# ut-vision/Rot-MVGaze

Measured on AMD Instinct MI355X. Metric: multi-view samples/sec (fwd+bwd), BxVx3x224x224, higher is better.
Workload: dtype f32; 1 GPU; C3: ResNet-50, V=4, B=128 per GPU, 3x224x224, fwd+loss+bwd; backbone=ResNet-50, views=4, batch_per_gpu=128, global_batch=128, image=3x224x224, parallelism=dp1, weights=random init, seed 0 (kaiming-normal convs, default Linear), rccl_ranks=1, step_launch=eager: every kernel queued from Python

## Files before the change

include/rotmvgaze.h:

```cpp
#ifndef ROTMVGAZE_H
#define ROTMVGAZE_H

#include <stddef.h>
#include <stdint.h>

#ifdef __cplusplus
extern "C" {
#endif

#define MVG_ABI_VERSION 13

int mvg_abi_version(void);
const char *mvg_last_error(void);
int mvg_device_cus(void);
int mvg_set_scratch(void *ptr, size_t bytes, void *stream);
size_t mvg_scratch_bytes(void);
void *mvg_stream_create_low_priority(void);
int mvg_set_reserved_cus(int n);

enum {
  MVG_K_CONV_FPROP = 0, MVG_K_CONV_DGRAD = 1, MVG_K_CONV_WGRAD = 2, MVG_K_WGRAD_REDUCE = 3,
  MVG_K_BN_FINALIZE = 4, MVG_K_BN_APPLY = 5, MVG_K_BN_BWD_REDUCE = 6, MVG_K_BN_BWD_APPLY = 7,
  MVG_K_POOL = 8, MVG_K_LAYOUT = 9, MVG_K_LINEAR_FPROP = 10, MVG_K_LINEAR_DGRAD = 11,
  MVG_K_LINEAR_WGRAD = 12, MVG_K_ROTCAT = 13, MVG_K_COLSUM = 14, MVG_K_LOSS = 15,
// ... 310 lines not shown
                            float *dz_out, float *mx, const float *gamma, float *dy_sinv, void *stream);
int mvg_bn_bwd_apply_split(const float *g, const float *y, const float *mean, const float *invstd, const float *gamma,
                           const float *s1, const float *s2, const float *relu_scale, const float *relu_shift,
                           int groups, int64_t rows_per_group, int c, void *dy_sp, const float *mx, float *dy_sinv,
                           int dy_sinv_ready, void *stream);
int mvg_bn_relu_maxpool_fwd_split(const float *y, const float *scale, const float *shift, void *pooled_sp,
                                  uint8_t *argmax, int groups, int n_per_group, int h, int w, int c, int ho, int wo,
                                  void *stream);
int mvg_avgpool_fwd_split(const void *x_sp, float *y, int n, int hw, int c, void *stream);
int mvg_act_scales(const void *items_dev, int n, float *slots, int n_slots, void *stream);
int mvg_bn_apply_split_scaled(const float *y, const float *scale, const float *shift, const void *residual, int residual_sp,
                              const float *res_scale, const float *res_shift, const float *res_sinv, int relu, void *out_sp,
                              const float *out_sinv, uint8_t *relu_bits, int groups, int64_t rows_per_group, int c,
                              void *stream);
int mvg_bn_relu_maxpool_fwd_split_scaled(const float *y, const float *scale, const float *shift, void *pooled_sp,
                                         const float *pooled_sinv, uint8_t *argmax, int groups, int n_per_group, int h, int w,
                                         int c, int ho, int wo, void *stream);
int mvg_avgpool_fwd_split_scaled(const void *x_sp, const float *x_sinv, float *y, int n, int hw, int c, void *stream);
int mvg_conv_dgrad_bn_partials_split(const mvg_conv_desc *d);
int mvg_conv_dgrad_split_bnreduce(const mvg_conv_desc *d, const void *dy_sp, const float *dy_sinv, const void *w_crsk_sp,
                                  const float *w_sinv, float *dx, const float *addend, const float *bn_y, const uint8_t *bn_bits,
                                  const float *bn_mean, const float *bn_invstd, const float *relu_scale, const float *relu_shift,
                                  float *partials, float *s1, float *s2, float *dgamma, float *dbeta, int accumulate,
                                  float *mx, const float *bn_gamma, float *dx_dy_sinv, void *stream);
int mvg_conv_dgrad_split_bnapply_bnreduce(const mvg_conv_desc *d, void *dy_sp, const float *dy_sinv, const float *dz, const float *y,
                                          const float *mean, const float *invstd, const float *gamma, const float *un_s1,
                                          const float *un_s2, int64_t rows_per_group, const void *w_crsk_sp, const float *w_sinv,
                                          float *dx, const float *addend, const float *bn_y, const uint8_t *bn_bits,
                                          const float *bn_mean, const float *bn_invstd, const float *relu_scale,
                                          const float *relu_shift, float *partials, float *s1, float *s2, float *dgamma, float *dbeta,
                                          int accumulate, float *mx, const float *bn_gamma, float *dx_dy_sinv, void *stream);
int mvg_conv_fprop_split_stages(const mvg_conv_desc *d);
int mvg_conv_dgrad_split_stages(const mvg_conv_desc *d, int fused_reduce);
int mvg_conv_fprop_split_bnapply(const mvg_conv_desc *d, void *out_sp, const float *out_sinv, const float *bn_y, const float *scale,
                                 const float *shift, const void *residual, int residual_sp, const float *res_scale,
                                 const float *res_shift, const float *res_sinv, uint8_t *relu_bits, const void *w_sp,
                                 const float *w_sinv, float *y, float *stats, void *stream);
int mvg_stem_rowwindow_split(const float *x_nhwc4, void *xw_sp, int64_t images, int h, int w, void *stream);
int mvg_stem_rowwindow_split_nchw(const float *x_nchw, void *xw_sp, int64_t images, int h, int w, void *stream);
int mvg_stem_fprop_split(const mvg_conv_desc *d, const void *xw_sp, const void *w_sp, const float *w_sinv, float *y, float *stats,
                         void *stream);
int mvg_stem_wgrad_splits_split(const mvg_conv_desc *d);
int mvg_stem_wgrad_split(const mvg_conv_desc *d, const void *xw_sp, const void *dy_sp, const float *dy_sinv, float *dw_rw,
                         float *workspace, int splits, int accumulate, void *stream);
int mvg_bn_relu_maxpool_bwd_reduce_split(const float *g_pooled, const uint8_t *argmax, const float *y, const float *mean,
                                         const float *invstd, const float *scale, const float *shift, int groups,
                                         int n_per_group, int h, int w, int c, int ho, int wo, float *s1, float *s2,
                                         float *dgamma, float *dbeta, int accumulate, float *workspace, float *mx, const float *gamma,
                                         float *dy_sinv, void *stream);
int mvg_bn_relu_maxpool_bwd_apply_split(const float *g_pooled, const uint8_t *argmax, const float *y, const float *mean,
                                        const float *invstd, const float *gamma, const float *scale, const float *shift,
                                        const float *s1, const float *s2, int groups, int n_per_group, int h, int w, int c,
                                        int ho, int wo, void *dy_sp, const float *mx, float *dy_sinv, int dy_sinv_ready, void *stream);
int mvg_conv_wgrad_splits_split(const mvg_conv_desc *d);
int mvg_conv_wgrad_split_tile(const mvg_conv_desc *d, int32_t *bm, int32_t *bn, int32_t *incremental);
int mvg_conv_wgrad_split(const mvg_conv_desc *d, const void *x_sp, const void *dy_sp, const float *dy_sinv, float *dw,
                         float *workspace, int splits, int accumulate, void *stream);
int mvg_conv_wgrad_split_slabs(const mvg_conv_desc *d, const void *x_sp, const void *dy_sp, const float *dy_sinv, float *workspace,
                               int splits, void *stream);
int mvg_conv_wgrad_split_xs(const mvg_conv_desc *d, const void *x_sp, const float *x_sinv, const void *dy_sp, const float *dy_sinv,
                            float *dw, float *workspace, int splits, int accumulate, void *stream);
int mvg_conv_wgrad_split_slabs_xs(const mvg_conv_desc *d, const void *x_sp, const float *x_sinv, const void *dy_sp,
                                  const float *dy_sinv, float *workspace, int splits, void *stream);
int mvg_wgrad_reduce_batch(const float *const *host_slabs, float *const *host_dw, const int64_t *host_n, const int32_t *host_splits,
                           const int32_t *host_accumulate, int n, void *stream);

// ... 53 lines not shown
```

rot-mvgaze_amd/_lib.py:

```python
from __future__ import annotations

import ctypes as C
import os

_HERE = os.path.dirname(os.path.abspath(__file__))
LIB_PATH = os.path.join(_HERE, "csrc", "librotmvgaze_hip.so")

K_FAMILIES = 18
ABI_VERSION = 13
SESSION_FP32, SESSION_BF16 = 0, 1


class ConvDesc(C.Structure):
    _fields_ = [(n, C.c_int32) for n in
                ("groups", "n", "h", "w", "cin", "cout", "r", "s", "stride", "pad", "ho", "wo")]

    @classmethod
    def make(cls, groups, n, h, w, cin, cout, k, stride, pad):
        ho = (h + 2 * pad - k) // stride + 1
        wo = (w + 2 * pad - k) // stride + 1
        return cls(groups, n, h, w, cin, cout, k, k, stride, pad, ho, wo)

    @classmethod
    def linear(cls, rows, fin, fout):
# ... 71 lines not shown
    "mvg_bn_apply": (_I, [_P, _P, _P, _P, _P, _P, _I, _P, _I, _I64, _I, _P]),
    "mvg_bn_bwd_reduce": (_I, [_P, _P, _P, _P, _P, _P, _P, _I, _I64, _I, _P, _P, _P, _P, _I, _P, _P, _P]),
    "mvg_split_f32": (_I, [_P, _P, _I64, _F, _P]),
    "mvg_merge_sp": (_I, [_P, _P, _I64, _F, _P]),
    "mvg_split_weights": (_I, [_D, _P, _P, _P, _P, _P, _P]),
    "mvg_weights_prep_batch": (_I, [_P, _I, _I, _I, _P]),
    "mvg_conv_stats_partials_split": (_I, [_D, C.POINTER(C.c_int32)]),
    "mvg_conv_fprop_split": (_I, [_D, _P, _P, _P, _P, _P, _P, _P]),
    "mvg_conv_fprop_split_affine": (_I, [_D, _P, _P, _P, _P, _P, _I, _P, _P, _P, _I, _I, _P]),
    "mvg_conv_dgrad_split": (_I, [_D, _P, _P, _P, _P, _P, _P, _P, _P]),
    "mvg_bn_apply_split": (_I, [_P, _P, _P, _P, _I, _P, _P, _I, _P, _P, _I, _I64, _I, _P]),
    "mvg_bn_bwd_apply_split": (_I, [_P, _P, _P, _P, _P, _P, _P, _P, _P, _I, _I64, _I, _P, _P, _P, _I, _P]),
    "mvg_bn_bwd_reduce_split": (_I, [_P, _P, _P, _P, _P, _P, _P, _I, _I64, _I, _P, _P, _P, _P, _I, _P, _P, _P, _P, _P, _P]),
    "mvg_bn_relu_maxpool_fwd_split": (_I, [_P, _P, _P, _P, _P, _I, _I, _I, _I, _I, _I, _I, _P]),
    "mvg_avgpool_fwd_split": (_I, [_P, _P, _I, _I, _I, _P]),
    "mvg_act_scales": (_I, [_P, _I, _P, _I, _P]),
    "mvg_bn_apply_split_scaled": (_I, [_P, _P, _P, _P, _I, _P, _P, _P, _I, _P, _P, _P, _I, _I64, _I, _P]),
    "mvg_bn_relu_maxpool_fwd_split_scaled": (_I, [_P, _P, _P, _P, _P, _P, _I, _I, _I, _I, _I, _I, _I, _P]),
    "mvg_avgpool_fwd_split_scaled": (_I, [_P, _P, _P, _I, _I, _I, _P]),
    "mvg_conv_wgrad_split_xs": (_I, [_D, _P, _P, _P, _P, _P, _P, _I, _I, _P]),
    "mvg_conv_wgrad_split_slabs_xs": (_I, [_D, _P, _P, _P, _P, _P, _I, _P]),
    "mvg_stem_rowwindow_split": (_I, [_P, _P, _I64, _I, _I, _P]),
    "mvg_stem_rowwindow_split_nchw": (_I, [_P, _P, _I64, _I, _I, _P]),
    "mvg_stem_fprop_split": (_I, [_D, _P, _P, _P, _P, _P, _P]),
    "mvg_stem_wgrad_splits_split": (_I, [_D]),
    "mvg_stem_wgrad_split": (_I, [_D, _P, _P, _P, _P, _P, _I, _I, _P]),
    "mvg_bn_relu_maxpool_bwd_reduce_split": (_I, [_P, _P, _P, _P, _P, _P, _P, _I, _I, _I, _I, _I, _I, _I, _P, _P, _P, _P, _I, _P, _P, _P, _P, _P]),
    "mvg_bn_relu_maxpool_bwd_apply_split": (_I, [_P, _P, _P, _P, _P, _P, _P, _P, _P, _P, _I, _I, _I, _I, _I, _I, _I, _P, _P, _P, _I, _P]),
    "mvg_conv_dgrad_bn_partials_split": (_I, [_D]),
    "mvg_conv_dgrad_split_bnreduce": (_I, [_D, _P, _P, _P, _P, _P, _P, _P, _P, _P, _P, _P, _P, _P, _P, _P, _P, _P, _I, _P, _P, _P, _P]),
    "mvg_conv_dgrad_split_bnapply_bnreduce": (_I, [_D] + [_P] * 9 + [_I64] + [_P] * 15 + [_I, _P, _P, _P, _P]),
    "mvg_conv_fprop_split_stages": (_I, [_D]),
    "mvg_conv_dgrad_split_stages": (_I, [_D, _I]),
    "mvg_conv_fprop_split_bnapply": (_I, [_D] + [_P] * 6 + [_I] + [_P] * 9),
    "mvg_conv_wgrad_splits_split": (_I, [_D]),
    "mvg_conv_wgrad_split_tile": (_I, [_D, C.POINTER(C.c_int32), C.POINTER(C.c_int32), C.POINTER(C.c_int32)]),
    "mvg_conv_wgrad_split": (_I, [_D, _P, _P, _P, _P, _P, _I, _I, _P]),
    "mvg_conv_wgrad_split_slabs": (_I, [_D, _P, _P, _P, _P, _I, _P]),
    "mvg_wgrad_reduce_batch": (_I, [C.POINTER(C.c_void_p), C.POINTER(C.c_void_p), C.POINTER(C.c_int64), C.POINTER(C.c_int32),
                                    C.POINTER(C.c_int32), _I, _P]),
    "mvg_bn_apply_bits": (_I, [_P, _P, _P, _P, _P, _P, _P, _P, _I, _I64, _I, _P]),
    "mvg_bn_bwd_reduce_bits": (_I, [_P, _P, _P, _P, _P, _I, _I64, _I, _P, _P, _P, _P, _I, _P, _P, _P]),
    "mvg_bn_apply_bits_bf16": (_I, [_P, _P, _P, _P, _P, _P, _P, _P, _I, _I64, _I, _P]),
    "mvg_bn_bwd_reduce_bits_bf16": (_I, [_P, _P, _P, _P, _P, _I, _I64, _I, _P, _P, _P, _P, _I, _P, _P, _P]),
    "mvg_bn_bwd_workspace_floats": (C.c_size_t, [_I, _I64, _I]),
    "mvg_bn_bwd_apply": (_I, [_P, _P, _P, _P, _P, _P, _P, _P, _P, _P, _I, _I64, _I, _P, _P, _P]),
    "mvg_maxpool3x3s2_fwd": (_I, [_P, _P, _P, _I, _I, _I, _I, _I, _I, _P]),
    "mvg_maxpool3x3s2_bwd": (_I, [_P, _P, _P, _I, _I, _I, _I, _I, _I, _P]),
    "mvg_bn_relu_maxpool_fwd": (_I, [_P, _P, _P, _P, _P, _I, _I, _I, _I, _I, _I, _I, _P]),
    "mvg_bn_relu_maxpool_bwd_reduce": (_I, [_P, _P, _P, _P, _P, _P, _P, _I, _I, _I, _I, _I, _I, _I, _P, _P, _P, _P, _I, _P,
                                            _P]),
    "mvg_bn_relu_maxpool_bwd_apply": (_I, [_P, _P, _P, _P, _P, _P, _P, _P, _P, _P, _I, _I, _I, _I, _I, _I, _I, _P, _P]),
    "mvg_bn_eval_bwd": (_I, [_P, _P, _P, _P, _P, _P, _P, _P, _P, _F, _I, _I64, _I, _P, _P, _P, _P, _I, _P, _P]),
    "mvg_bn_eval_bwd_workspace_floats": (C.c_size_t, [_I, _I64, _I]),
    "mvg_bn_relu_maxpool_eval_bwd": (_I, [_P, _P, _P, _P, _P, _P, _P, _P, _F, _I, _I, _I, _I, _I, _I, _I, _P, _P, _P, _I, _P,
                                          _P]),
    "mvg_avgpool_fwd": (_I, [_P, _P, _I, _I, _I, _P]),
    "mvg_avgpool_bwd": (_I, [_P, _P, _I, _I, _I, _P]),
    "mvg_nchw_to_nhwc4": (_I, [_P, _P, _I, _I, _I, _I, _P]),
    "mvg_nhwc4_to_nchw": (_I, [_P, _P, _I, _I, _I, _I, _P]),
    "mvg_preprocess_u8hwc": (_I, [_P, _P, _I, _I, _I, _F, _F, _F, _F, _F, _F, _I, _P]),
    "mvg_gaze_lp_loss": (_I, [_P, _P, _I, _I, _P, _P, _P]),
    "mvg_preprocess_u8hwc_resize": (_I, [_P, _P, _I, _I, _I, _I, _I, _F, _F, _F, _F, _F, _F, _I, _P]),
    "mvg_multi_erase_nchw": (_I, [_P, _P, _P, _I, _I, _I, _I, _I, _P]),
    "mvg_augment_u8hwc": (_I, [_P, _P, _P, _P, _P, _P, _P, _I, _I, _I, _I, _F, _F, _F, _F, _F, _F, _I, _P]),
    "mvg_rotation_matrix_2d": (_I, [_P, _P, _I, _I, _P]),
# ... 104 lines not shown
```

rot-mvgaze_amd/csrc/conv_split.hip:

```cpp
#include "bf16_tile.h"
#include "elem.h"

namespace mvg {

typedef _Float16 f16x8 __attribute__((ext_vector_type(8)));

#define SPLIT_ONE(PA, PB, av, bv, acc)                                                                         \
  _Pragma("unroll") for (int i = 0; i < TM; ++i) _Pragma("unroll") for (int j = 0; j < TN; ++j)                \
      acc[i][j] = __builtin_amdgcn_mfma_f32_32x32x16_f16(av[PA][i], bv[PB][j], acc[i][j], 0, 0, 0);
#define SPLIT_PRODUCTS(av, bv, acc) SPLIT_ONE(0, 1, av, bv, acc) SPLIT_ONE(1, 0, av, bv, acc) SPLIT_ONE(0, 0, av, bv, acc)

constexpr int SP_BM = 128, SP_BK = 32;

__global__ __launch_bounds__(256) void split_f32_kernel(const float4 *__restrict__ x, uint4 *__restrict__ out, long long n8, float scale) {
  const long long stride = (long long)gridDim.x * 256;
  for (long long i = (long long)blockIdx.x * 256 + threadIdx.x; i < n8; i += stride) {
    const float4 lo = x[2 * i], hi = x[2 * i + 1];
    const float v[8] = {lo.x * scale, lo.y * scale, lo.z * scale, lo.w * scale, hi.x * scale, hi.y * scale, hi.z * scale, hi.w * scale};
    uint4 q1, q2;
    split2_chunk(v, q1, q2);
    out[2 * i] = q1;
    out[2 * i + 1] = q2;
  }
}
// ... 182 lines not shown
#pragma unroll
        for (int q = 0; q < 2; ++q) {
          const int idx = threadIdx.x + 256 * q, cl = idx >> 3, o8 = idx & 7;
          float v[8];
#pragma unroll
          for (int k = 0; k < 8; ++k) v[k] = tile[o8 * 8 + k][cl];
          *reinterpret_cast<uint4 *>(wt + (long long)(c0 + cl) * cout + o0 + o8 * 8) =
              make_uint4(bf16_pack2(v[0], v[1]), bf16_pack2(v[2], v[3]), bf16_pack2(v[4], v[5]), bf16_pack2(v[6], v[7]));
        }
      }
    }
    return;
  }
  for (long long i = (long long)blockIdx.x * 256 + threadIdx.x; i < total; i += (long long)gridDim.x * 256) {
    const int c = (int)(i % cin_pad);
    const long long t = i / cin_pad;
    const int tap = (int)(t % rs), o = (int)(t / rs);
    const float v = c < cin ? w[((long long)o * rs + tap) * cin + c] : 0.f;
    const __bf16 b = (__bf16)v;
    const unsigned short u = __builtin_bit_cast(unsigned short, b);
    wk[i] = u;
    if (wt) wt[((long long)c * rs + tap) * cout + o] = u;
  }
}

typedef float f32x4 __attribute__((ext_vector_type(4)));

#define SPLIT16_ONE(PA, PB)                                                                       \
  _Pragma("unroll") for (int i = 0; i < TM; ++i) _Pragma("unroll") for (int j = 0; j < TN; ++j)   \
      acc[i][j] = __builtin_amdgcn_mfma_f32_16x16x32_f16(av[PA][i], bv[PB][j], acc[i][j], 0, 0, 0);

__device__ __forceinline__ int sp_row_swz(int R) { return ((R >> 1) & 1) | (((R >> 2) & 1) << 2); }

enum AForm : int { A_DMA = 0, A_DY = 1, A_OUT_SP = 2, A_OUT_AFFINE = 3 };
constexpr int BNA_MAX_C = 512;

__device__ __forceinline__ void unpack8(const float4 (&v)[2], float (&o)[8]) {
  o[0] = v[0].x; o[1] = v[0].y; o[2] = v[0].z; o[3] = v[0].w; o[4] = v[1].x; o[5] = v[1].y; o[6] = v[1].z; o[7] = v[1].w;
}

struct DyFormer {
  static constexpr int TABLES = 5;
  __amdgpu_buffer_rsrc_t rs_dz, rs_y;
  float inv_rows, dsc;
  float4 dzv[2][2], yv[2][2];
  float mu[8], is[8], ga[8], sa[8], sb[8];
  static __device__ __forceinline__ void stage(float *t, const IgemmParams &p, int g, int C, int tid) {
    for (int i = tid; i < C; i += 256) {
      const long long gc = (long long)g * C + i;
      t[i] = p.bna_mean[gc];
      t[C + i] = p.bna_invstd[gc];
      t[2 * C + i] = p.bna_gamma[i];
      t[3 * C + i] = p.bna_s1[gc];
      t[4 * C + i] = p.bna_s2[gc];
    }
  }
  __device__ __forceinline__ DyFormer(const IgemmParams &p, long long grow0, long long rows_per_group, int C)
      : rs_dz(make_rsrc(p.bna_dz + grow0 * C, 4ll * rows_per_group * C)), rs_y(make_rsrc(p.bna_y + grow0 * C, 4ll * rows_per_group * C)),
        inv_rows(p.bna_inv_rows), dsc(1.f / *p.a_sinv) {}
  __device__ __forceinline__ void load(int i, unsigned off) {
    dzv[i][0] = buf_ld16(rs_dz, off);
    dzv[i][1] = buf_ld16(rs_dz, off + 16u);
    yv[i][0] = buf_ld16(rs_y, off);
    yv[i][1] = buf_ld16(rs_y, off + 16u);
  }
  __device__ __forceinline__ void consts(const float *kc, int C) {
    ld8(kc, mu);
// ... 264 lines not shown
static int validate_split(const mvg_conv_desc *d) {
  if (validate(d)) return 2;
  MVG_REQUIRE(d->cin % 32 == 0 && d->cout % 32 == 0, "split conv: cin and cout must be multiples of 32 (got %d, %d)", d->cin,
              d->cout);
  MVG_REQUIRE(d->r * d->s <= 32, "split conv: at most 32 filter taps");
  return 0;
}

static int split_tile_rows(int ncols, int taps, long long rows) { return (ncols < 128 && taps > 1 && rows >= 65536) ? 256 : SP_BM; }

struct SplitPlan { int bm, bn, kt_max; long long tiles; bool pipelined; };
static int split_conv_stages(const SplitPlan &pl) { return (pl.pipelined && pl.bn == 128 && pl.bm == SP_BM) ? 2 : 1; }
static SplitPlan split_plan(int ncols, int taps, long long rows, int groups, bool lin, IgemmClass *cls, int ncls) {
  SplitPlan pl;
  pl.bm = lin ? SP_BM : split_tile_rows(ncols, taps, rows);
  pl.bn = ncols >= 128 ? 128 : 64;
  if (lin && pl.bn == 128 && ncls == 1) {
    const long long t128 = (long long)groups * ceil_div(cls[0].rows_per_group, pl.bm) * ceil_div(ncols, 128);
    if (2 * t128 <= compute_cus()) pl.bn = 64;
  }
  pl.tiles = 0, pl.kt_max = 0;
  for (int i = 0; i < ncls; ++i) {
    IgemmClass &c = cls[i];
    c.mtiles_per_group = ceil_div(c.rows_per_group, pl.bm);
    c.KT = ceil_div(c.ktotal, SP_BK);
    c.tile0 = (int)pl.tiles;
    pl.tiles += (long long)groups * c.mtiles_per_group * ceil_div(ncols, pl.bn);
    pl.kt_max = c.KT > pl.kt_max ? c.KT : pl.kt_max;
  }
  pl.pipelined = pl.tiles <= 2LL * compute_cus() || (pl.tiles <= 4LL * compute_cus() && pl.kt_max >= 48);
  return pl;
}

template <bool DGRAD>
static int launch_igemm_split(IgemmParams &p, hipStream_t st, bool lin, int taps, long long rows, AForm af = A_DMA, bool ranged = false) {
  const SplitPlan pl = split_plan(p.ncols, taps, rows, p.groups, lin, p.cls, p.ncls);
  const int bm = pl.bm, bn = pl.bn;
  const bool pipelined = pl.pipelined;
  p.ntiles = ceil_div(p.ncols, bn);
  p.splits = 1;
  p.sk_tiles = 0;
  p.bn_parts = 0;
  for (int i = 0; i < p.ncls; ++i) {
    IgemmClass &c = p.cls[i];
    c.korder = c.ntaps > 1 ? 1 : 0;
    c.per_div = make_fastdiv((unsigned)(c.ntaps > 0 ? c.ntaps : 1));
    c.unit0 = 0;
    c.part0 = p.bn_parts;
    p.bn_parts += c.mtiles_per_group;
    MVG_REQUIRE((c.ntaps >= 1 || (DGRAD && p.bn_part)) && c.ntaps <= 32 && c.ktotal % SP_BK == 0, "split conv: class shape not covered");
  }
  MVG_REQUIRE(pl.tiles < (1LL << 31), "split conv: grid too large");
  if (pl.tiles <= 0) return 0;
  p.nt_out = (!lin && !(DGRAD && p.cls_step == 2)) ? 1 : 0;
  dim3 grid((unsigned)pl.tiles), block(256);
  if (af != A_DMA) {
    MVG_REQUIRE(!lin && bm == SP_BM && p.ntiles == 1 && p.ncls == 1 && DGRAD == (af == A_DY), "split conv: the operand-forming loaders take one column tile");
    if constexpr (DGRAD) {
      if (bn == 128) hipLaunchKernelGGL((igemm_split16_kernel<128, true, false, 2, 1, A_DY>), grid, block, 0, st, p);
      else hipLaunchKernelGGL((igemm_split16_kernel<64, true, false, 2, 1, A_DY>), grid, block, 0, st, p);
      return check_launch("conv_dgrad_split_bnapply");
    } else {
      if (bn == 128 && af == A_OUT_AFFINE) hipLaunchKernelGGL((igemm_split16_kernel<128, false, false, 2, 1, A_OUT_AFFINE>), grid, block, 0, st, p);
      else if (bn == 128) hipLaunchKernelGGL((igemm_split16_kernel<128, false, false, 2, 1, A_OUT_SP>), grid, block, 0, st, p);
      else if (af == A_OUT_AFFINE) hipLaunchKernelGGL((igemm_split16_kernel<64, false, false, 2, 1, A_OUT_AFFINE>), grid, block, 0, st, p);
      else hipLaunchKernelGGL((igemm_split16_kernel<64, false, false, 2, 1, A_OUT_SP>), grid, block, 0, st, p);
      return check_launch("conv_fprop_split_bnapply");
    }
  }
  if (ranged) {
    MVG_REQUIRE(!DGRAD && !lin && p.out_sp && p.out_absmax, "split conv: the range record goes with a forward that stores sp");
    if constexpr (!DGRAD) {
      if (bm == 256) hipLaunchKernelGGL((igemm_split16_ranged_kernel<64, 4>), grid, block, 0, st, p);
      else if (split_conv_stages(pl) == 2) hipLaunchKernelGGL((igemm_split16_ranged_kernel<128, 2, 2>), grid, block, 0, st, p);
      else if (bn == 128) hipLaunchKernelGGL((igemm_split16_ranged_kernel<128>), grid, block, 0, st, p);
      else hipLaunchKernelGGL((igemm_split16_ranged_kernel<64>), grid, block, 0, st, p);
    }
    return check_launch("conv_fprop_split_ranged");
  }
  if (lin) {
    if (bn == 128 && pipelined) hipLaunchKernelGGL((igemm_split16_kernel<128, DGRAD, true, 2, 2>), grid, block, 0, st, p);
    else if (bn == 128) hipLaunchKernelGGL((igemm_split16_kernel<128, DGRAD, true>), grid, block, 0, st, p);
    else if (pipelined) hipLaunchKernelGGL((igemm_split16_kernel<64, DGRAD, true, 2, 2>), grid, block, 0, st, p);
    else hipLaunchKernelGGL((igemm_split16_kernel<64, DGRAD, true>), grid, block, 0, st, p);
  } else if (bm == 256) hipLaunchKernelGGL((igemm_split16_kernel<64, DGRAD, false, 4>), grid, block, 0, st, p);
  else if (split_conv_stages(pl) == 2) hipLaunchKernelGGL((igemm_split16_kernel<128, DGRAD, false, 2, 2>), grid, block, 0, st, p);
  else if (bn == 128) hipLaunchKernelGGL((igemm_split16_kernel<128, DGRAD>), grid, block, 0, st, p);
  else hipLaunchKernelGGL((igemm_split16_kernel<64, DGRAD>), grid, block, 0, st, p);
  return check_launch(DGRAD ? "conv_dgrad_split" : "conv_fprop_split");
}

}

using namespace mvg;

extern "C" {

int mvg_split_f32(const float *x, void *out_sp, int64_t n, float scale, void *stream) {
  MVG_REQUIRE(x && out_sp && n >= 0 && n % 8 == 0, "split_f32: null argument or n %% 8 != 0");
  MVG_REQUIRE(scale > 0.f, "split_f32: scale must be positive (a power of two keeps the round trip exact)");
  if (n == 0) return 0;
  hipStream_t st = (hipStream_t)stream;
  ProfScope ps(MVG_K_LAYOUT, st, 0.0, (4.0 + SP_BYTES) * (double)n);
  long long blocks = (n / 8 + 255) / 256;
  if (blocks > 8192) blocks = 8192;
  hipLaunchKernelGGL(split_f32_kernel, dim3((unsigned)blocks), dim3(256), 0, st, (const float4 *)x, (uint4 *)out_sp, (long long)(n / 8), scale);
  return check_launch("split_f32");
}

int mvg_split_f32_ranged(const float *x, void *out_sp, int64_t n, float scale, uint32_t *range_word, void *stream) {
  MVG_REQUIRE(x && out_sp && range_word && n >= 0 && n % 8 == 0, "split_f32_ranged: null argument or n %% 8 != 0");
  MVG_REQUIRE(scale > 0.f, "split_f32_ranged: scale must be positive (a power of two keeps the round trip exact)");
  if (n == 0) return 0;
  hipStream_t st = (hipStream_t)stream;
  ProfScope ps(MVG_K_LAYOUT, st, 0.0, (4.0 + SP_BYTES) * (double)n);
  long long blocks = (n / 8 + 255) / 256;
  if (blocks > 8192) blocks = 8192;
  hipLaunchKernelGGL(split_f32_ranged_kernel, dim3((unsigned)blocks), dim3(256), 0, st, (const float4 *)x, (uint4 *)out_sp, (long long)(n / 8), scale,
// ... 211 lines not shown
    p.bna_invstd = bna->invstd;
    p.bna_gamma = bna->gamma;
    p.bna_s1 = bna->s1;
    p.bna_s2 = bna->s2;
    p.bna_inv_rows = 1.0f / (float)bna->rows_per_group;
  }
  if (dgrad_geometry(p, d, SP_BYTES, SP_BYTES, "split conv")) return 2;
  MVG_REQUIRE((long long)d->n * d->h * d->w * d->cin < (1ll << 31), "split conv: a group of dx exceeds 2^31 elements");
  const double flops = 2.0 * d->groups * (double)d->n * d->ho * d->wo * d->cout * d->r * d->s * d->cin;
  const double bytes = (double)SP_BYTES * (d->groups * (double)d->n * d->ho * d->wo * d->cout + (double)d->cout * d->r * d->s * d->cin) +
                       (bnf ? 8.25 : 4.0) * d->groups * (double)d->n * d->h * d->w * d->cin +
                       (bna ? 8.0 : 0.0) * d->groups * (double)d->n * d->ho * d->wo * d->cout;
  const bool lin = d->r == 1 && d->s == 1 && d->h == 1 && d->w == 1;
  ProfScope ps(lin ? MVG_K_LINEAR_DGRAD : MVG_K_CONV_DGRAD, (hipStream_t)stream, flops, bytes);
  if (int e = dgrad_classes(p, d, bnf != nullptr, 4, dx, addend, (hipStream_t)stream)) return e;
  if (p.ncls == 0) return 0;
  return launch_igemm_split<true>(p, (hipStream_t)stream, lin_kernel, d->r * d->s, (long long)d->n * d->h * d->w, bna ? A_DY : A_DMA);
}

int mvg_conv_dgrad_split(const mvg_conv_desc *d, const void *dy_sp, const float *dy_sinv, const void *w_crsk_sp, const float *w_sinv,
                         float *dx, const float *addend, const void *relu_mask_sp, void *stream) {
  MVG_REQUIRE(!relu_mask_sp || d->stride == 1, "dgrad_split: the sp ReLU mask is for stride-1 launches (Linear layers)");
  return dgrad_split_impl(d, dy_sp, dy_sinv, w_crsk_sp, w_sinv, dx, addend, stream, nullptr, relu_mask_sp);
}

int mvg_conv_dgrad_split_stages(const mvg_conv_desc *d, int fused_reduce) {
  if (validate_split(d)) return -1;
  IgemmParams p;
  memset(&p, 0, sizeof(p));
  if (dgrad_geometry(p, d, SP_BYTES, SP_BYTES, "split conv")) return -1;
  DgradDropped dropped;
  dgrad_plan_classes(p, d, fused_reduce != 0, dropped);
  return split_conv_stages(split_plan(p.ncols, d->r * d->s, (long long)d->n * d->h * d->w, p.groups, false, p.cls, p.ncls));
}

int mvg_conv_dgrad_bn_partials_split(const mvg_conv_desc *d) {
  if (validate_split(d)) return -1;
  return dgrad_bn_partials(d, split_tile_rows(d->cin, d->r * d->s, (long long)d->n * d->h * d->w));
}

static int dgrad_split_bnreduce_impl(const char *who, const mvg_conv_desc *d, const void *dy_sp, const float *dy_sinv, const void *w_crsk_sp,
                                     const float *w_sinv, float *dx, const float *addend, const float *bn_y, const uint8_t *bn_bits,
                                     const float *bn_mean, const float *bn_invstd, const float *relu_scale, const float *relu_shift,
                                     float *partials, float *s1, float *s2, float *dgamma, float *dbeta, int accumulate, float *mx,
                                     const float *bn_gamma, float *dx_dy_sinv, void *stream, const SplitBnApply *bna) {
  MVG_REQUIRE(bn_y && bn_mean && bn_invstd && partials && s1 && s2, "%s: null argument", who);
  MVG_REQUIRE((bn_gamma == nullptr) == (dx_dy_sinv == nullptr) && (!dx_dy_sinv || mx), "%s: bn_gamma, dx_dy_sinv (and mx) go together", who);
  MVG_REQUIRE(!(bn_bits && relu_scale) && ((relu_scale == nullptr) == (relu_shift == nullptr)),
              "%s: give the ReLU mask either as bits or as (relu_scale, relu_shift)", who);
  const int P = mvg_conv_dgrad_bn_partials_split(d);
  MVG_REQUIRE(P > 0, "%s: bad descriptor", who);
  const SplitBnFuse f = {bn_y, bn_bits, bn_mean, bn_invstd, relu_scale, relu_shift, partials, mx ? 3 : 2};
  if (dgrad_split_impl(d, dy_sp, dy_sinv, w_crsk_sp, w_sinv, dx, addend, stream, &f, nullptr, false, nullptr, bna)) return 1;
  ProfScope ps(MVG_K_BN_BWD_REDUCE, (hipStream_t)stream, 0.0, 8.0 * d->groups * (double)P * d->cin);
  return bn_bwd_finalize_launch(partials, d->groups, P, d->cin, s1, s2, dgamma, dbeta, accumulate, (hipStream_t)stream, mx, nullptr, nullptr,
                                bn_gamma, bn_invstd, (long long)d->n * d->h * d->w, dx_dy_sinv);
}

int mvg_conv_dgrad_split_bnreduce(const mvg_conv_desc *d, const void *dy_sp, const float *dy_sinv, const void *w_crsk_sp,
                                  const float *w_sinv, float *dx, const float *addend, const float *bn_y, const uint8_t *bn_bits,
                                  const float *bn_mean, const float *bn_invstd, const float *relu_scale, const float *relu_shift,
                                  float *partials, float *s1, float *s2, float *dgamma, float *dbeta, int accumulate,
                                  float *mx, const float *bn_gamma, float *dx_dy_sinv, void *stream) {
  return dgrad_split_bnreduce_impl("dgrad_split_bnreduce", d, dy_sp, dy_sinv, w_crsk_sp, w_sinv, dx, addend, bn_y, bn_bits, bn_mean, bn_invstd,
                                   relu_scale, relu_shift, partials, s1, s2, dgamma, dbeta, accumulate, mx, bn_gamma, dx_dy_sinv, stream, nullptr);
}
// ... 238 lines not shown
```

rot-mvgaze_amd/csrc/conv_split_igemm.inc:

```
#ifndef MVG_SPLIT_RNG
#error "conv_split_igemm.inc: define MVG_SPLIT_RNG (0 or 1) before including"
#endif

#if MVG_SPLIT_RNG
template <int BN, int WGM = 2, int STAGES = 1>
__global__ __launch_bounds__(256, STAGES == 2 ? 2 : WGM == 4 ? 3 : 4) void igemm_split16_ranged_kernel(IgemmParams p) {
  constexpr bool DGRAD = false, LIN = false;
  constexpr AForm AF = A_DMA;
#else
template <int BN, bool DGRAD, bool LIN = false, int WGM = 2, int STAGES = 1, AForm AF = A_DMA>
__global__ __launch_bounds__(256, STAGES == 2 ? 2 : (DGRAD || WGM == 4 || AF != A_DMA) ? 3 : 4) void igemm_split16_kernel(IgemmParams p) {
#endif
  constexpr int BM = 64 * WGM, WGN = 4 / WGM, NW = 4;
  static_assert(WGM == 2 || (WGM == 4 && BN == 64), "tiles: 128 x BN (2 x 2 waves) or 256 x 64 (4 x 1)");
  static_assert(STAGES == 1 || STAGES == 2, "one LDS stage, or the two-stage pipeline");
  static_assert(AF == A_DMA || (DGRAD == (AF == A_DY) && !LIN && WGM == 2 && STAGES == 1),
                "operand-forming loaders: dy in backward-data, the block output in forward; 128-row tiles, one stage");
  using Former = std::conditional_t<AF == A_DY, DyFormer, OutFormer<AF == A_OUT_AFFINE>>;
  constexpr int WTM = BM / WGM, WTN = BN / WGN;
  constexpr int TM = WTM / 16, TN = WTN / 16;
  constexpr int SLOTS = 4 * SP_NP;
  constexpr int ROWB = 16 * SLOTS, ROWS = BM + BN, STAGE_B = ROWS * ROWB;
  constexpr int NQ = ROWS * SLOTS / 64;
  constexpr int QA = BM * SLOTS / 64;
  constexpr int A_PER = QA / NW, B_PER = (NQ - QA) / NW;
  static_assert(QA % NW == 0 && (NQ - QA) % NW == 0, "whole instructions per wave");
  constexpr int EPI_B = bf16_epilogue_bytes<BM, BN, WGM, DGRAD>();
  constexpr int INFO_OFF = STAGES * STAGE_B > EPI_B ? STAGES * STAGE_B : EPI_B;
  constexpr int BNK_OFF = INFO_OFF + BM * 8;
  constexpr int SMEM_B = BNK_OFF + (AF != A_DMA ? Former::TABLES : 0) * BNA_MAX_C * 4;
  __shared__ __attribute__((aligned(16))) unsigned char smem[SMEM_B];

  const int tid = threadIdx.x;
  const int lane = tid & 63, wave = __builtin_amdgcn_readfirstlane(tid >> 6);
  const int wm = wave / WGN, wn = wave % WGN;
  const int nwg = gridDim.x;
  const int wg_all = p.no_remap ? (int)blockIdx.x : xcd_remap(blockIdx.x, nwg);
  int ci = 0;
  for (int i = 1; i < p.ncls; ++i) ci += wg_all >= p.cls[i].tile0;
  const IgemmClass &c = p.cls[ci];
  const int wg = wg_all - c.tile0;
  const int ntile = wg % p.ntiles;
  const int mt_all = wg / p.ntiles;
  const int g = mt_all / c.mtiles_per_group;
  const int mtile = mt_all - g * c.mtiles_per_group;
  const int KT = c.KT;
  const int ohw = c.out_h * c.out_w;

  uint2 *rowinfo = reinterpret_cast<uint2 *>(smem + INFO_OFF);
  if (tid < BM) {
    const long long m = (long long)mtile * BM + tid;
    const bool ok = m < c.rows_per_group;
    const int mm = ok ? (int)m : 0;
    const int img = (int)fdiv((unsigned)mm, c.ohw_div);
    const int rem = mm - img * ohw;
    const int oy = (int)fdiv((unsigned)rem, c.ow_div), ox = rem - oy * c.out_w;
    const int y0 = DGRAD ? oy + c.cls_cy : oy * p.stride - p.pad;
    const int x0 = DGRAD ? ox + c.cls_cx : ox * p.stride_w - p.pad_w;
    const unsigned base = (unsigned)(img * p.src_img_stride * SP_BYTES) + (unsigned)((y0 * p.src_w + x0) * p.src_c) * (unsigned)SP_BYTES;
    unsigned msk = 0;
    for (int t = 0; t < c.ntaps; ++t) {
      const int fr = (int)fdiv((unsigned)t, c.tap_ns_div), fs = t - fr * c.tap_ns;
      const int iy = DGRAD ? y0 - fr : y0 + fr;
      const int ix = DGRAD ? x0 - fs : x0 + fs;
      msk |= (unsigned)(((unsigned)iy < (unsigned)p.src_h) & ((unsigned)ix < (unsigned)p.src_w)) << t;
    }
    rowinfo[tid] = make_uint2(base, ok ? msk : 0u);
  }
  if constexpr (AF != A_DMA) Former::stage(reinterpret_cast<float *>(smem + BNK_OFF), p, g, p.src_c, tid);
  __syncthreads();
  unsigned a_base[A_PER], a_vmask[A_PER], b_base[B_PER];
#pragma unroll
  for (int i = 0; i < A_PER; ++i) {
    const int sl = (wave + NW * i) * 64 + lane;
    const int row = sl / SLOTS, j = (sl % SLOTS) ^ sp_row_swz(row);
    const uint2 ri = rowinfo[row];
    a_base[i] = ri.x + 16u * (unsigned)j;
    a_vmask[i] = ri.y;
  }
#pragma unroll
  for (int i = 0; i < B_PER; ++i) {
    const int sl = (wave + NW * (A_PER + i)) * 64 + lane - BM * SLOTS;
    const int row = sl / SLOTS, j = (sl % SLOTS) ^ sp_row_swz(row);
    const int n = ntile * BN + row;
    b_base[i] = pred_off(((unsigned)n * (unsigned)p.b_row_len) * (unsigned)SP_BYTES + 16u * (unsigned)j, n < p.ncols);
  }
  const __amdgpu_buffer_rsrc_t rs_a =
      make_rsrc(reinterpret_cast<const char *>(p.a) + (long long)g * p.imgs_per_group * p.src_img_stride * SP_BYTES, p.a_group_bytes);
  const __amdgpu_buffer_rsrc_t rs_b = make_rsrc(p.b, p.b_bytes);
  typedef __attribute__((address_space(3))) void *lds_vp;

  auto issue = [&](int kt, int stage_off) {
    int kstart = kt * SP_BK;
    if (c.korder) {
      const int cblk = (int)fdiv((unsigned)kt, c.per_div), rem = kt - cblk * c.ntaps;
      kstart = (rem << p.src_c_shift) + cblk * SP_BK;
    }
    const int ks = __builtin_amdgcn_readfirstlane(kstart);
    const int tap_u = c.ntaps > 1 ? (ks >> p.src_c_shift) : 0;
    const int chb = ks - (tap_u << p.src_c_shift);
    const int fru = (int)fdiv((unsigned)tap_u, c.tap_ns_div), fsu = tap_u - fru * c.tap_ns;
    const int disp = (fru * p.src_w + fsu) * p.src_c;
// ... 18 lines not shown
  f32x4 acc[TM][TN];
#pragma unroll
  for (int i = 0; i < TM; ++i)
#pragma unroll
    for (int j = 0; j < TN; ++j)
#pragma unroll
      for (int e = 0; e < 4; ++e) acc[i][j][e] = 0.f;

  const int cc_l = lane >> 4;
  int a_off[TM][SP_NP], b_off[TN][SP_NP];
#pragma unroll
  for (int i = 0; i < TM; ++i) {
    const int R = wm * WTM + i * 16 + (lane & 15);
#pragma unroll
    for (int pc = 0; pc < SP_NP; ++pc) a_off[i][pc] = R * ROWB + (((2 * cc_l + pc) ^ sp_row_swz(R)) << 4);
  }
#pragma unroll
  for (int j = 0; j < TN; ++j) {
    const int R = wn * WTN + j * 16 + (lane & 15);
#pragma unroll
    for (int pc = 0; pc < SP_NP; ++pc) b_off[j][pc] = (BM + R) * ROWB + (((2 * cc_l + pc) ^ sp_row_swz(R)) << 4);
  }

  auto load_frags = [&](const unsigned char *stage, f16x8 (&av)[SP_NP][TM], f16x8 (&bv)[SP_NP][TN]) {
#pragma unroll
    for (int pc = 0; pc < SP_NP; ++pc) {
#pragma unroll
      for (int i = 0; i < TM; ++i) av[pc][i] = *reinterpret_cast<const f16x8 *>(stage + a_off[i][pc]);
#pragma unroll
      for (int j = 0; j < TN; ++j) bv[pc][j] = *reinterpret_cast<const f16x8 *>(stage + b_off[j][pc]);
    }
  };
  auto products = [&](const f16x8 (&av)[SP_NP][TM], const f16x8 (&bv)[SP_NP][TN]) { SPLIT16_ONE(0, 1) SPLIT16_ONE(1, 0) SPLIT16_ONE(0, 0) };
  if constexpr (AF != A_DMA) {
    const int C = p.src_c;
    const int a_cc = tid & 3, a_r0 = tid >> 2;
    const long long grow0 = (long long)g * c.rows_per_group;
    Former f(p, grow0, c.rows_per_group, C);
    uint4 *a_out = reinterpret_cast<uint4 *>(const_cast<float *>(p.a)) + grow0 * C / 4;
    bool a_ok[2];
    unsigned a_goff[2];
#pragma unroll
    for (int i = 0; i < 2; ++i) {
      const long long m = (long long)mtile * BM + a_r0 + 64 * i;
      a_ok[i] = m < c.rows_per_group;
      a_goff[i] = pred_off((unsigned)m * (unsigned)C * 4u + 32u * (unsigned)a_cc, a_ok[i]);
    }
    auto a_load = [&](int kt) {
#pragma unroll
      for (int i = 0; i < 2; ++i) f.load(i, a_goff[i] + 128u * (unsigned)kt);
    };
    constexpr bool PREFETCH = BN == 64;
    if (PREFETCH) a_load(0);
    for (int kt = 0; kt < KT; ++kt) {
      issue(kt, 0);
      if (!PREFETCH) a_load(kt);
      uint4 q[2][SP_NP];
      f.consts(reinterpret_cast<const float *>(smem + BNK_OFF) + kt * SP_BK + a_cc * 8, C);
#pragma unroll
      for (int i = 0; i < 2; ++i) {
        float o[8];
        f.form(i, a_ok[i], o);
        split2_chunk(o, q[i][0], q[i][1]);
        const int R = a_r0 + 64 * i;
#pragma unroll
        for (int pc = 0; pc < SP_NP; ++pc)
          *reinterpret_cast<uint4 *>(smem + R * ROWB + (((2 * a_cc + pc) ^ sp_row_swz(R)) << 4)) = q[i][pc];
      }
      asm volatile("s_waitcnt vmcnt(0)" ::: "memory");
      __syncthreads();
#pragma unroll
      for (int i = 0; i < 2; ++i)
        if (a_ok[i]) {
          const unsigned off = a_goff[i] + 128u * (unsigned)kt;
          uint4 *dst = a_out + (off >> 4);
          dst[0] = q[i][0];
          dst[1] = q[i][1];
          f.store_extra(i, off);
        }
      if (PREFETCH && kt + 1 < KT) a_load(kt + 1);
      {
        f16x8 av[SP_NP][TM], bv[SP_NP][TN];
        load_frags(smem, av, bv);
        products(av, bv);
      }
      __syncthreads();
    }
  } else if constexpr (STAGES == 1) {
    for (int kt = 0; kt < KT; ++kt) {
      issue(kt, 0);
      asm volatile("s_waitcnt vmcnt(0)" ::: "memory");
      __syncthreads();
      {
        f16x8 av[SP_NP][TM], bv[SP_NP][TN];
        load_frags(smem, av, bv);
        products(av, bv);
      }
      __syncthreads();
    }
  } else {
    constexpr int G = A_PER + B_PER;
    if (KT > 0) issue(0, 0);
    if (KT > 1) {
      issue(1, STAGE_B);
      asm volatile("s_waitcnt vmcnt(%0)\n\ts_barrier" ::"n"(G) : "memory");
    } else {
      asm volatile("s_waitcnt vmcnt(0)\n\ts_barrier" ::: "memory");
    }
    f16x8 a0[SP_NP][TM], b0[SP_NP][TN], a1[SP_NP][TM], b1[SP_NP][TN];
    load_frags(smem, a0, b0);
    int cur = 0;
    auto step = [&](int kt, const f16x8 (&ca)[SP_NP][TM], const f16x8 (&cb)[SP_NP][TN], f16x8 (&na)[SP_NP][TM], f16x8 (&nb)[SP_NP][TN]) {
      if (kt + 1 < KT) {
        asm volatile("s_waitcnt vmcnt(0) lgkmcnt(0)\n\ts_barrier" ::: "memory");
        if (kt + 2 < KT) issue(kt + 2, cur);
        cur ^= STAGE_B;
        load_frags(smem + cur, na, nb);
      }
      products(ca, cb);
    };
// ... 14 lines not shown
```

rot-mvgaze_amd/ops.py:

```python
from __future__ import annotations

import ctypes as C
from typing import Optional

import torch

from ._lib import ConvDesc, K_FAMILIES, ProfEntry, check, lib

Tensor = torch.Tensor


def _p(t: Optional[Tensor]):
    if t is None:
        return None
    assert t.is_cuda and t.dtype in _PTR_DTYPES, (t.device, t.dtype)
    return t.data_ptr()


_PTR_DTYPES = frozenset((torch.float32, torch.int32, torch.uint8, torch.int16, torch.bfloat16, torch.float16))
_workspaces = {}
_MAX_WORKSPACES = 8
_raw_stream = getattr(torch._C, "_cuda_getCurrentRawStream", None)


# ... 194 lines not shown
    stat = torch.empty(2, dtype=torch.float32, device=w.device)
    items = torch.empty(64, dtype=torch.uint8, device=w.device)
    check(lib().mvg_split_weights(C.byref(d), _p(w), _p(wk), _p(wt), _p(stat), _p(items), _s()), "split_weights")
    wk.sinv = stat[1:2]
    if wt is not None:
        wt.sinv = stat[1:2]
    return wk, wt


def weights_prep_batch(table: Tensor, n: int, mode: int, blocks_per_item: int = 0):
    assert table.is_cuda and table.dtype == torch.int64 and table.is_contiguous() and table.shape == (n, 6)
    check(lib().mvg_weights_prep_batch(C.c_void_p(table.data_ptr()), n, mode, blocks_per_item, _s()), "weights_prep_batch")


def conv_stats_partials_split(d: ConvDesc):
    rpp = C.c_int32(0)
    n = lib().mvg_conv_stats_partials_split(C.byref(d), C.byref(rpp))
    if n < 0:
        check(1, "conv_stats_partials_split")
    return n, rpp.value


def conv_fprop_split(d: ConvDesc, x_sp: Tensor, w_sp: Tensor, y: Tensor, stats: Optional[Tensor] = None):
    check(lib().mvg_conv_fprop_split(C.byref(d), _p(x_sp), _sinv(x_sp), _p(w_sp), _sinv(w_sp), _p(y), _p(stats), _s()), "conv_fprop_split")


def conv_fprop_split_stages(d: ConvDesc) -> int:
    n = lib().mvg_conv_fprop_split_stages(C.byref(d))
    if n < 0:
        check(1, "conv_fprop_split_stages")
    return n


def conv_dgrad_split_stages(d: ConvDesc, fused_reduce: bool = False) -> int:
    n = lib().mvg_conv_dgrad_split_stages(C.byref(d), int(fused_reduce))
    if n < 0:
        check(1, "conv_dgrad_split_stages")
    return n


def conv_wgrad_split_tile(d: ConvDesc):
    bm, bn, incr = C.c_int32(0), C.c_int32(0), C.c_int32(0)
    if lib().mvg_conv_wgrad_split_tile(C.byref(d), C.byref(bm), C.byref(bn), C.byref(incr)) != 0:
        check(1, "conv_wgrad_split_tile")
    return bm.value, bn.value, bool(incr.value)


def conv_fprop_split_bnapply(d: ConvDesc, out_sp: Tensor, bn_y, scale, shift, residual, w_sp: Tensor, y: Tensor,
                             stats: Optional[Tensor] = None, residual_affine=None, bits: Optional[Tensor] = None):
    assert bits is None or (bits.dtype == torch.uint8 and bits.numel() == d.groups * d.n * d.h * d.w * d.cin // 4)
    rs, rh = residual_affine if residual_affine is not None else (None, None)
    res_sp = is_sp(residual)
    check(lib().mvg_conv_fprop_split_bnapply(C.byref(d), _p(out_sp), _sinv(out_sp), _p(bn_y), _p(scale), _p(shift), _p(residual), int(res_sp),
                                             _p(rs), _p(rh), _sinv(residual) if res_sp else None, _p(bits), _p(w_sp), _sinv(w_sp), _p(y),
                                             _p(stats), _s()), "conv_fprop_split_bnapply")


def conv_fprop_split_affine(d: ConvDesc, x_sp: Tensor, w_sp: Tensor, out: Tensor, scale: Tensor, shift: Tensor,
                            residual: Optional[Tensor], relu: bool):
    assert getattr(residual, "sinv", None) is None, "conv_fprop_split_affine: the residual is read unscaled"
    check(lib().mvg_conv_fprop_split_affine(C.byref(d), _p(x_sp), _sinv(x_sp), _p(w_sp), _sinv(w_sp), _p(out), int(is_sp(out)), _p(scale),
                                            _p(shift), _p(residual), int(is_sp(residual)), int(relu), _s()), "conv_fprop_split_affine")


def conv_fprop_split_affine_ranged(d: ConvDesc, x_sp: Tensor, w_sp: Tensor, out: Tensor, scale: Tensor, shift: Tensor,
                                   residual: Optional[Tensor], relu: bool, range_word: Tensor):
# ... 540 lines not shown
```

Before: 1689 samples/s.

## Add filter-row strip A-loader for 3x3 stride-1 split implicit-GEMM convs

Adds an A_ROW operand mode for the 256x64 split implicit-GEMM conv kernel on 3x3, stride-1, pad-1 convolutions. For each channel block and filter row it loads one contiguous pixel strip (BM+2 rows) into LDS once. The three horizontal taps then read it at shifted row offsets, with per-tap masking from the row-info bits. B tiles for the next tap are double-buffered, so A traffic for three taps is cut to roughly one load. The path is on by default through a global flag, and a query API is exposed. Costs are extra LDS for the strip, per-element masking selects in the fragment loads, and a full vmcnt(0) wait plus barrier after each tap.

```diff
diff --git a/include/rotmvgaze.h b/include/rotmvgaze.h
--- a/include/rotmvgaze.h
+++ b/include/rotmvgaze.h
@@ -366,6 +366,8 @@
                                           int accumulate, float *mx, const float *bn_gamma, float *dx_dy_sinv, void *stream);
 int mvg_conv_fprop_split_stages(const mvg_conv_desc *d);
 int mvg_conv_dgrad_split_stages(const mvg_conv_desc *d, int fused_reduce);
+int mvg_set_split_taprow(int on);
+int mvg_conv_split_taprow(const mvg_conv_desc *d, int dgrad);
 int mvg_conv_fprop_split_bnapply(const mvg_conv_desc *d, void *out_sp, const float *out_sinv, const float *bn_y, const float *scale,
                                  const float *shift, const void *residual, int residual_sp, const float *res_scale,
                                  const float *res_shift, const float *res_sinv, uint8_t *relu_bits, const void *w_sp,
diff --git a/rot-mvgaze_amd/_lib.py b/rot-mvgaze_amd/_lib.py
--- a/rot-mvgaze_amd/_lib.py
+++ b/rot-mvgaze_amd/_lib.py
@@ -127,6 +127,8 @@
     "mvg_conv_dgrad_split_bnapply_bnreduce": (_I, [_D] + [_P] * 9 + [_I64] + [_P] * 15 + [_I, _P, _P, _P, _P]),
     "mvg_conv_fprop_split_stages": (_I, [_D]),
     "mvg_conv_dgrad_split_stages": (_I, [_D, _I]),
+    "mvg_set_split_taprow": (_I, [_I]),
+    "mvg_conv_split_taprow": (_I, [_D, _I]),
     "mvg_conv_fprop_split_bnapply": (_I, [_D] + [_P] * 6 + [_I] + [_P] * 9),
     "mvg_conv_wgrad_splits_split": (_I, [_D]),
     "mvg_conv_wgrad_split_tile": (_I, [_D, C.POINTER(C.c_int32), C.POINTER(C.c_int32), C.POINTER(C.c_int32)]),
diff --git a/rot-mvgaze_amd/csrc/conv_split.hip b/rot-mvgaze_amd/csrc/conv_split.hip
--- a/rot-mvgaze_amd/csrc/conv_split.hip
+++ b/rot-mvgaze_amd/csrc/conv_split.hip
@@ -238,7 +238,7 @@
 
 __device__ __forceinline__ int sp_row_swz(int R) { return ((R >> 1) & 1) | (((R >> 2) & 1) << 2); }
 
-enum AForm : int { A_DMA = 0, A_DY = 1, A_OUT_SP = 2, A_OUT_AFFINE = 3 };
+enum AForm : int { A_DMA = 0, A_DY = 1, A_OUT_SP = 2, A_OUT_AFFINE = 3, A_ROW = 4 };
 constexpr int BNA_MAX_C = 512;
 
 __device__ __forceinline__ void unpack8(const float4 (&v)[2], float (&o)[8]) {
@@ -569,6 +569,16 @@
   return pl;
 }
 
+static int g_split_taprow = 1;
+template <bool DGRAD>
+static bool split_taprow(const SplitPlan &pl, const IgemmParams &p) {
+  const IgemmClass &c = p.cls[0];
+  if (!g_split_taprow || pl.bm != 256 || p.ncls != 1 || p.r != 3 || p.s != 3 || p.stride != 1 || p.pad != 1 || p.src_c % SP_BK != 0) return false;
+  if (c.ntaps != 9 || c.tap_ns != 3 || p.src_h != c.out_h || p.src_w != c.out_w) return false;
+  if (DGRAD) return p.cls_step == 1 && p.tap_step == 1 && c.tap_r0 == 0 && c.tap_s0 == 0 && c.cls_cy == 1 && c.cls_cx == 1;
+  return p.stride_w == 1 && p.pad_w == 1;
+}
+
 template <bool DGRAD>
 static int launch_igemm_split(IgemmParams &p, hipStream_t st, bool lin, int taps, long long rows, AForm af = A_DMA, bool ranged = false) {
   const SplitPlan pl = split_plan(p.ncols, taps, rows, p.groups, lin, p.cls, p.ncls);
@@ -620,7 +630,8 @@
     else if (bn == 128) hipLaunchKernelGGL((igemm_split16_kernel<128, DGRAD, true>), grid, block, 0, st, p);
     else if (pipelined) hipLaunchKernelGGL((igemm_split16_kernel<64, DGRAD, true, 2, 2>), grid, block, 0, st, p);
     else hipLaunchKernelGGL((igemm_split16_kernel<64, DGRAD, true>), grid, block, 0, st, p);
-  } else if (bm == 256) hipLaunchKernelGGL((igemm_split16_kernel<64, DGRAD, false, 4>), grid, block, 0, st, p);
+  } else if (bm == 256 && split_taprow<DGRAD>(pl, p)) hipLaunchKernelGGL((igemm_split16_kernel<64, DGRAD, false, 4, 1, A_ROW>), grid, block, 0, st, p);
+  else if (bm == 256) hipLaunchKernelGGL((igemm_split16_kernel<64, DGRAD, false, 4>), grid, block, 0, st, p);
   else if (split_conv_stages(pl) == 2) hipLaunchKernelGGL((igemm_split16_kernel<128, DGRAD, false, 2, 2>), grid, block, 0, st, p);
   else if (bn == 128) hipLaunchKernelGGL((igemm_split16_kernel<128, DGRAD>), grid, block, 0, st, p);
   else hipLaunchKernelGGL((igemm_split16_kernel<64, DGRAD>), grid, block, 0, st, p);
@@ -898,6 +909,26 @@
   DgradDropped dropped;
   dgrad_plan_classes(p, d, fused_reduce != 0, dropped);
   return split_conv_stages(split_plan(p.ncols, d->r * d->s, (long long)d->n * d->h * d->w, p.groups, false, p.cls, p.ncls));
+}
+
+int mvg_set_split_taprow(int on) {
+  g_split_taprow = on != 0;
+  return 0;
+}
+
+int mvg_conv_split_taprow(const mvg_conv_desc *d, int dgrad) {
+  if (d != nullptr && (d->r != 3 || d->s != 3 || d->stride != 1 || d->pad != 1)) return 0;
+  if (validate_split(d)) return -1;
+  IgemmParams p;
+  memset(&p, 0, sizeof(p));
+  if (dgrad) {
+    if (dgrad_geometry(p, d, SP_BYTES, SP_BYTES, "split conv")) return -1;
+    DgradDropped dropped;
+    dgrad_plan_classes(p, d, false, dropped);
+    return split_taprow<true>(split_plan(p.ncols, d->r * d->s, (long long)d->n * d->h * d->w, p.groups, false, p.cls, p.ncls), p);
+  }
+  if (fprop_geometry(p, d, SP_BYTES, SP_BYTES, "split conv")) return -1;
+  return split_taprow<false>(split_plan(p.ncols, d->r * d->s, p.rows_per_group, p.groups, false, p.cls, p.ncls), p);
 }
 
 int mvg_conv_dgrad_bn_partials_split(const mvg_conv_desc *d) {
diff --git a/rot-mvgaze_amd/csrc/conv_split_igemm.inc b/rot-mvgaze_amd/csrc/conv_split_igemm.inc
--- a/rot-mvgaze_amd/csrc/conv_split_igemm.inc
+++ b/rot-mvgaze_amd/csrc/conv_split_igemm.inc
@@ -14,8 +14,10 @@
   constexpr int BM = 64 * WGM, WGN = 4 / WGM, NW = 4;
   static_assert(WGM == 2 || (WGM == 4 && BN == 64), "tiles: 128 x BN (2 x 2 waves) or 256 x 64 (4 x 1)");
   static_assert(STAGES == 1 || STAGES == 2, "one LDS stage, or the two-stage pipeline");
-  static_assert(AF == A_DMA || (DGRAD == (AF == A_DY) && !LIN && WGM == 2 && STAGES == 1),
+  constexpr bool FORMED = AF == A_DY || AF == A_OUT_SP || AF == A_OUT_AFFINE;
+  static_assert(!FORMED || (DGRAD == (AF == A_DY) && !LIN && WGM == 2 && STAGES == 1),
                 "operand-forming loaders: dy in backward-data, the block output in forward; 128-row tiles, one stage");
+  static_assert(AF != A_ROW || (!LIN && WGM == 4 && STAGES == 1), "filter-row strips: the 256 x 64 tile, one stage");
   using Former = std::conditional_t<AF == A_DY, DyFormer, OutFormer<AF == A_OUT_AFFINE>>;
   constexpr int WTM = BM / WGM, WTN = BN / WGN;
   constexpr int TM = WTM / 16, TN = WTN / 16;
@@ -26,9 +28,11 @@
   constexpr int A_PER = QA / NW, B_PER = (NQ - QA) / NW;
   static_assert(QA % NW == 0 && (NQ - QA) % NW == 0, "whole instructions per wave");
   constexpr int EPI_B = bf16_epilogue_bytes<BM, BN, WGM, DGRAD>();
-  constexpr int INFO_OFF = STAGES * STAGE_B > EPI_B ? STAGES * STAGE_B : EPI_B;
+  constexpr int STRIP_ROWS = (BM + 2 + 7) / 8 * 8, STRIP_B = STRIP_ROWS * ROWB, BTILE_B = BN * ROWB;
+  constexpr int LOAD_B = AF == A_ROW ? STRIP_B + 2 * BTILE_B : STAGES * STAGE_B;
+  constexpr int INFO_OFF = LOAD_B > EPI_B ? LOAD_B : EPI_B;
   constexpr int BNK_OFF = INFO_OFF + BM * 8;
-  constexpr int SMEM_B = BNK_OFF + (AF != A_DMA ? Former::TABLES : 0) * BNA_MAX_C * 4;
+  constexpr int SMEM_B = BNK_OFF + (FORMED ? Former::TABLES : 0) * BNA_MAX_C * 4;
   __shared__ __attribute__((aligned(16))) unsigned char smem[SMEM_B];
 
   const int tid = threadIdx.x;
@@ -67,7 +71,7 @@
     }
     rowinfo[tid] = make_uint2(base, ok ? msk : 0u);
   }
-  if constexpr (AF != A_DMA) Former::stage(reinterpret_cast<float *>(smem + BNK_OFF), p, g, p.src_c, tid);
+  if constexpr (FORMED) Former::stage(reinterpret_cast<float *>(smem + BNK_OFF), p, g, p.src_c, tid);
   __syncthreads();
   unsigned a_base[A_PER], a_vmask[A_PER], b_base[B_PER];
 #pragma unroll
@@ -152,7 +156,7 @@
     }
   };
   auto products = [&](const f16x8 (&av)[SP_NP][TM], const f16x8 (&bv)[SP_NP][TN]) { SPLIT16_ONE(0, 1) SPLIT16_ONE(1, 0) SPLIT16_ONE(0, 0) };
-  if constexpr (AF != A_DMA) {
+  if constexpr (FORMED) {
     const int C = p.src_c;
     const int a_cc = tid & 3, a_r0 = tid >> 2;
     const long long grow0 = (long long)g * c.rows_per_group;
@@ -206,6 +210,71 @@
       }
       __syncthreads();
     }
+  } else if constexpr (AF == A_ROW) {
+    const int pshift = p.src_c_shift + 2;
+    const unsigned npix = (unsigned)(p.imgs_per_group * p.src_h * p.src_w);
+    const int s_row0 = 8 * wave + (lane >> 3);
+    const unsigned s_slot = 16u * (unsigned)((lane & 7) ^ sp_row_swz(s_row0));
+    const int s_pix0 = mtile * BM - 1 + s_row0;
+    constexpr int SQ = STRIP_ROWS / 8;
+    unsigned rmask[TM];
+#pragma unroll
+    for (int i = 0; i < TM; ++i) rmask[i] = rowinfo[wm * WTM + i * 16 + (lane & 15)].y;
+    auto issue_strip = [&](int cb, int fr) {
+      const int dpix = (DGRAD ? 1 - fr : fr - 1) * p.src_w;
+      const unsigned chb = (unsigned)(cb * SP_BK * SP_BYTES);
+#pragma unroll
+      for (int i = 0; i < (SQ + NW - 1) / NW; ++i) {
+        if (NW * i + NW > SQ && wave + NW * i >= SQ) break;
+        const int pix = s_pix0 + 8 * NW * i + dpix;
+        const unsigned off = ((unsigned)pix << pshift) + chb + s_slot;
+        __builtin_amdgcn_raw_ptr_buffer_load_lds(rs_a, (lds_vp)(smem + (wave + NW * i) * 1024), 16, (int)pred_off(off, (unsigned)pix < npix), 0, 0, 0);
+      }
+    };
+    auto issue_b = [&](int cb, int fr, int fs, int boff) {
+      const int tap = DGRAD ? (c.tap_r0 + p.tap_step * fr) * p.s + c.tap_s0 + p.tap_step * fs : fr * c.tap_ns + fs;
+      const unsigned kb = (unsigned)((tap << p.src_c_shift) + cb * SP_BK) * (unsigned)SP_BYTES;
+#pragma unroll
+      for (int i = 0; i < B_PER; ++i)
+        __builtin_amdgcn_raw_ptr_buffer_load_lds(rs_b, (lds_vp)(smem + boff + (wave + NW * i) * 1024), 16, (int)(b_base[i] + kb), 0, 0, 0);
+    };
+    int cb = 0, fr = 0;
+    for (int kt = 0; kt < KT; kt += 3) {
+      issue_strip(cb, fr);
+      issue_b(cb, fr, 0, STRIP_B);
+      asm volatile("s_waitcnt vmcnt(0)" ::: "memory");
+      __syncthreads();
+#pragma unroll
+      for (int fs = 0; fs < 3; ++fs) {
+        if (fs < 2) issue_b(cb, fr, fs + 1, STRIP_B + ((fs + 1) & 1) * BTILE_B);
+        {
+          f16x8 av[SP_NP][TM], bv[SP_NP][TN];
+          const unsigned char *bt = smem + STRIP_B + (fs & 1) * BTILE_B - BM * ROWB;
+          const int tbit = fr * 3 + fs;
+#pragma unroll
+          for (int i = 0; i < TM; ++i) {
+            const int R = wm * WTM + i * 16 + (lane & 15) + (DGRAD ? 2 - fs : fs);
+            const bool ok = ((rmask[i] >> tbit) & 1u) != 0u;
+#pragma unroll
+            for (int pc = 0; pc < SP_NP; ++pc) {
+              const u32x4 v = *reinterpret_cast<const u32x4 *>(smem + R * ROWB + (((2 * cc_l + pc) ^ sp_row_swz(R)) << 4));
+              u32x4 z;
+#pragma unroll
+              for (int e = 0; e < 4; ++e) z[e] = ok ? v[e] : 0u;
+              av[pc][i] = __builtin_bit_cast(f16x8, z);
+            }
+          }
+#pragma unroll
+          for (int pc = 0; pc < SP_NP; ++pc)
+#pragma unroll
+            for (int j = 0; j < TN; ++j) bv[pc][j] = *reinterpret_cast<const f16x8 *>(bt + b_off[j][pc]);
+          products(av, bv);
+        }
+        if (fs < 2) asm volatile("s_waitcnt vmcnt(0)" ::: "memory");
+        __syncthreads();
+      }
+      if (++fr == 3) fr = 0, ++cb;
+    }
   } else if constexpr (STAGES == 1) {
     for (int kt = 0; kt < KT; ++kt) {
       issue(kt, 0);
diff --git a/rot-mvgaze_amd/ops.py b/rot-mvgaze_amd/ops.py
--- a/rot-mvgaze_amd/ops.py
+++ b/rot-mvgaze_amd/ops.py
@@ -250,6 +250,17 @@
     return n
 
 
+def set_split_taprow(on: bool):
+    check(lib().mvg_set_split_taprow(int(bool(on))), "set_split_taprow")
+
+
+def conv_split_taprow(d: ConvDesc, dgrad: bool = False) -> bool:
+    n = lib().mvg_conv_split_taprow(C.byref(d), int(bool(dgrad)))
+    if n < 0:
+        check(1, "conv_split_taprow")
+    return n == 1
+
+
 def conv_dgrad_split_stages(d: ConvDesc, fused_reduce: bool = False) -> int:
     n = lib().mvg_conv_dgrad_split_stages(C.byref(d), int(fused_reduce))
     if n < 0:
```

Result: no change. 1683 samples/s (-0.4%).
